# NVIDIA/spark-rapids-ml

Measured on NVIDIA H100. Metric: kmeans_fit_samples_per_sec, higher is better.
Workload: dtype f32

## Files before the change

profile_fused.py:

```python
from __future__ import annotations

import argparse
import json
import os
import sys

ROOT = os.path.dirname(os.path.abspath(__file__))
if ROOT not in sys.path:
    sys.path.insert(0, ROOT)

from bench_pca import _card

CONSUMER = ["X wait", "centre wait", "hand-off wait", "A load + split", "MMA issue + drain", "epilogue", "sort",
            "column sums"]
PRODUCER = ["X slot wait", "centre stage wait", "issue"]
TILE_ROWS = 128


def main() -> None:
    ap = argparse.ArgumentParser()
    ap.add_argument("--rows", type=int, default=10_000_000)
    ap.add_argument("--d", type=int, default=128)
    ap.add_argument("--k", type=int, default=64)
    ap.add_argument("--warmup", type=int, default=3)
    a = ap.parse_args()

    import numpy as np
    import torch

    from bench import make_blobs_device
    from spark_rapids_ml_b200 import _native

    dev = torch.device("cuda", 0)
    X, _ = make_blobs_device(torch, dev, a.rows, a.d, a.k, 0)
    C0 = X[: a.k].clone()
    with _native.Context(0) as ctx:
        ctx.set_option("kernel_path", 2)
        ctx.kmeans_lloyd(X, C0.clone(), a.warmup, -1.0)
        ctx.set_option("profile_fused", 1)
        ctx.kmeans_lloyd(X, C0.clone(), 1, -1.0)
        ctx.set_option("profile_fused", 0)
        prof = ctx.fused_profile().astype(np.float64)
    grid = prof.shape[0]
    ntiles = -(-a.rows // TILE_ROWS)
    tiles = np.array([len(range(b, ntiles, grid)) for b in range(grid)], dtype=np.float64)
    per_tile = prof / tiles[:, None, None]
    cons = per_tile[:, :8, :].mean(axis=(0, 1))
    prod = per_tile[:, 8, :3].mean(axis=0)
    rec = {"shape": {"n": a.rows, "d": a.d, "k": a.k}, "grid": grid, "tiles_per_cta": float(tiles.mean()),
           "consumer_cycles_per_tile": {nm: round(float(v)) for nm, v in zip(CONSUMER, cons)},
           "consumer_total": round(float(cons.sum())),
           "producer_cycles_per_tile": {nm: round(float(v)) for nm, v in zip(PRODUCER, prod)},
           "producer_total": round(float(prod.sum())), **_card()}
    print(f"{rec['gpu']}, power limit {rec['power_limit']}; grid {grid}, {rec['tiles_per_cta']:.1f} tiles per CTA")
    print("consumer warps (mean), cycles per tile:")
    for nm, v in rec["consumer_cycles_per_tile"].items():
        print(f"  {nm:20s} {v:8d}")
    print(f"  {'total':20s} {rec['consumer_total']:8d}")
    print("producer warp, cycles per tile:")
    for nm, v in rec["producer_cycles_per_tile"].items():
        print(f"  {nm:20s} {v:8d}")
    print(f"  {'total':20s} {rec['producer_total']:8d}")
    print(json.dumps(rec))


if __name__ == "__main__":
    main()
# ... 1 lines not shown
```

spark_rapids_ml_b200/csrc/b2k_ptx.cuh:

```cuda
#pragma once
__device__ __forceinline__ uint32_t smem_u32(const void* p) { return (uint32_t)__cvta_generic_to_shared(p); }

__device__ __forceinline__ void mbar_init(uint32_t bar, uint32_t count) {
  asm volatile("mbarrier.init.shared::cta.b64 [%0], %1;" ::"r"(bar), "r"(count) : "memory");
}
__device__ __forceinline__ void mbar_arrive(uint32_t bar) {
  asm volatile("mbarrier.arrive.shared::cta.b64 _, [%0];" ::"r"(bar) : "memory");
}
__device__ __forceinline__ void mbar_expect_tx(uint32_t bar, uint32_t bytes) {
  asm volatile("mbarrier.arrive.expect_tx.shared::cta.b64 _, [%0], %1;" ::"r"(bar), "r"(bytes) : "memory");
}
__device__ __forceinline__ uint32_t mbar_try_wait(uint32_t bar, uint32_t parity) {
  uint32_t ok;
  asm volatile(
      "{\n\t.reg .pred p;\n\t"
      "mbarrier.try_wait.parity.shared::cta.b64 p, [%1], %2, %3;\n\t"
      "selp.u32 %0, 1, 0, p;\n\t}"
      : "=r"(ok)
      : "r"(bar), "r"(parity), "r"(200000u)
      : "memory");
  return ok;
}
__device__ __forceinline__ void mbar_wait_nocall(uint32_t bar, uint32_t parity) {
  uint32_t spins = 0;
// ... 142 lines not shown
      : "+f"(d[0]), "+f"(d[1]), "+f"(d[2]), "+f"(d[3]), "+f"(d[4]), "+f"(d[5]), "+f"(d[6]), "+f"(d[7]), "+f"(d[8]), "+f"(d[9]), "+f"(d[10]), "+f"(d[11]), "+f"(d[12]), "+f"(d[13]), "+f"(d[14]), "+f"(d[15]), "+f"(d[16]), "+f"(d[17]), "+f"(d[18]), "+f"(d[19]), "+f"(d[20]), "+f"(d[21]), "+f"(d[22]), "+f"(d[23]), "+f"(d[24]), "+f"(d[25]), "+f"(d[26]), "+f"(d[27]), "+f"(d[28]), "+f"(d[29]), "+f"(d[30]), "+f"(d[31]), "+f"(d[32]), "+f"(d[33]), "+f"(d[34]), "+f"(d[35]), "+f"(d[36]), "+f"(d[37]), "+f"(d[38]), "+f"(d[39]), "+f"(d[40]), "+f"(d[41]), "+f"(d[42]), "+f"(d[43]), "+f"(d[44]), "+f"(d[45]), "+f"(d[46]), "+f"(d[47]), "+f"(d[48]), "+f"(d[49]), "+f"(d[50]), "+f"(d[51]), "+f"(d[52]), "+f"(d[53]), "+f"(d[54]), "+f"(d[55]), "+f"(d[56]), "+f"(d[57]), "+f"(d[58]), "+f"(d[59]), "+f"(d[60]), "+f"(d[61]), "+f"(d[62]), "+f"(d[63]), "+f"(d[64]), "+f"(d[65]), "+f"(d[66]), "+f"(d[67]), "+f"(d[68]), "+f"(d[69]), "+f"(d[70]), "+f"(d[71]), "+f"(d[72]), "+f"(d[73]), "+f"(d[74]), "+f"(d[75]), "+f"(d[76]), "+f"(d[77]), "+f"(d[78]), "+f"(d[79]), "+f"(d[80]), "+f"(d[81]), "+f"(d[82]), "+f"(d[83]), "+f"(d[84]), "+f"(d[85]), "+f"(d[86]), "+f"(d[87]), "+f"(d[88]), "+f"(d[89]), "+f"(d[90]), "+f"(d[91]), "+f"(d[92]), "+f"(d[93]), "+f"(d[94]), "+f"(d[95]), "+f"(d[96]), "+f"(d[97]), "+f"(d[98]), "+f"(d[99]), "+f"(d[100]), "+f"(d[101]), "+f"(d[102]), "+f"(d[103]), "+f"(d[104]), "+f"(d[105]), "+f"(d[106]), "+f"(d[107]), "+f"(d[108]), "+f"(d[109]), "+f"(d[110]), "+f"(d[111]), "+f"(d[112]), "+f"(d[113]), "+f"(d[114]), "+f"(d[115]), "+f"(d[116]), "+f"(d[117]), "+f"(d[118]), "+f"(d[119]), "+f"(d[120]), "+f"(d[121]), "+f"(d[122]), "+f"(d[123]), "+f"(d[124]), "+f"(d[125]), "+f"(d[126]), "+f"(d[127])
      : "l"(da), "l"(db), "r"(scale_d));
}
template <int N> __device__ __forceinline__ void wgmma_tf32(float (&d)[N / 2], uint64_t da, uint64_t db, uint32_t sd) {
  if constexpr (N == 16) wgmma_tf32_n16(d, da, db, sd);
  else if constexpr (N == 32) wgmma_tf32_n32(d, da, db, sd);
  else if constexpr (N == 64) wgmma_tf32_n64(d, da, db, sd);
  else if constexpr (N == 128) wgmma_tf32_n128(d, da, db, sd);
  else wgmma_tf32_n256(d, da, db, sd);
}

__device__ __forceinline__ void wgmma_tf32_rs_n16(float (&d)[8], const uint32_t (&a)[4], uint64_t db, uint32_t scale_d) {
  asm volatile(
      "{\n\t.reg .pred p;\n\t"
      "setp.ne.b32 p, %13, 0;\n\t"
      "wgmma.mma_async.sync.aligned.m64n16k8.f32.tf32.tf32 "
      "{%0, %1, %2, %3, %4, %5, %6, %7}, {%8, %9, %10, %11}, %12, p, 1, 1;\n\t}"
      : "+f"(d[0]), "+f"(d[1]), "+f"(d[2]), "+f"(d[3]), "+f"(d[4]), "+f"(d[5]), "+f"(d[6]), "+f"(d[7])
      : "r"(a[0]), "r"(a[1]), "r"(a[2]), "r"(a[3]), "l"(db), "r"(scale_d));
}
__device__ __forceinline__ void wgmma_tf32_rs_n32(float (&d)[16], const uint32_t (&a)[4], uint64_t db, uint32_t scale_d) {
  asm volatile(
      "{\n\t.reg .pred p;\n\t"
      "setp.ne.b32 p, %21, 0;\n\t"
      "wgmma.mma_async.sync.aligned.m64n32k8.f32.tf32.tf32 "
      "{%0, %1, %2, %3, %4, %5, %6, %7, %8, %9, %10, %11, %12, %13, %14, %15}, {%16, %17, %18, %19}, %20, p, 1, 1;\n\t}"
      : "+f"(d[0]), "+f"(d[1]), "+f"(d[2]), "+f"(d[3]), "+f"(d[4]), "+f"(d[5]), "+f"(d[6]), "+f"(d[7]), "+f"(d[8]), "+f"(d[9]), "+f"(d[10]), "+f"(d[11]), "+f"(d[12]), "+f"(d[13]), "+f"(d[14]), "+f"(d[15])
      : "r"(a[0]), "r"(a[1]), "r"(a[2]), "r"(a[3]), "l"(db), "r"(scale_d));
}
__device__ __forceinline__ void wgmma_tf32_rs_n64(float (&d)[32], const uint32_t (&a)[4], uint64_t db, uint32_t scale_d) {
  asm volatile(
      "{\n\t.reg .pred p;\n\t"
      "setp.ne.b32 p, %37, 0;\n\t"
      "wgmma.mma_async.sync.aligned.m64n64k8.f32.tf32.tf32 "
      "{%0, %1, %2, %3, %4, %5, %6, %7, %8, %9, %10, %11, %12, %13, %14, %15, %16, %17, %18, %19, %20, %21, %22, %23, %24, %25, %26, %27, %28, %29, %30, %31}, {%32, %33, %34, %35}, %36, p, 1, 1;\n\t}"
      : "+f"(d[0]), "+f"(d[1]), "+f"(d[2]), "+f"(d[3]), "+f"(d[4]), "+f"(d[5]), "+f"(d[6]), "+f"(d[7]), "+f"(d[8]), "+f"(d[9]), "+f"(d[10]), "+f"(d[11]), "+f"(d[12]), "+f"(d[13]), "+f"(d[14]), "+f"(d[15]), "+f"(d[16]), "+f"(d[17]), "+f"(d[18]), "+f"(d[19]), "+f"(d[20]), "+f"(d[21]), "+f"(d[22]), "+f"(d[23]), "+f"(d[24]), "+f"(d[25]), "+f"(d[26]), "+f"(d[27]), "+f"(d[28]), "+f"(d[29]), "+f"(d[30]), "+f"(d[31])
      : "r"(a[0]), "r"(a[1]), "r"(a[2]), "r"(a[3]), "l"(db), "r"(scale_d));
}
__device__ __forceinline__ void wgmma_tf32_rs_n128(float (&d)[64], const uint32_t (&a)[4], uint64_t db, uint32_t scale_d) {
  asm volatile(
      "{\n\t.reg .pred p;\n\t"
      "setp.ne.b32 p, %69, 0;\n\t"
      "wgmma.mma_async.sync.aligned.m64n128k8.f32.tf32.tf32 "
      "{%0, %1, %2, %3, %4, %5, %6, %7, %8, %9, %10, %11, %12, %13, %14, %15, %16, %17, %18, %19, %20, %21, %22, %23, %24, %25, %26, %27, %28, %29, %30, %31, %32, %33, %34, %35, %36, %37, %38, %39, %40, %41, %42, %43, %44, %45, %46, %47, %48, %49, %50, %51, %52, %53, %54, %55, %56, %57, %58, %59, %60, %61, %62, %63}, {%64, %65, %66, %67}, %68, p, 1, 1;\n\t}"
      : "+f"(d[0]), "+f"(d[1]), "+f"(d[2]), "+f"(d[3]), "+f"(d[4]), "+f"(d[5]), "+f"(d[6]), "+f"(d[7]), "+f"(d[8]), "+f"(d[9]), "+f"(d[10]), "+f"(d[11]), "+f"(d[12]), "+f"(d[13]), "+f"(d[14]), "+f"(d[15]), "+f"(d[16]), "+f"(d[17]), "+f"(d[18]), "+f"(d[19]), "+f"(d[20]), "+f"(d[21]), "+f"(d[22]), "+f"(d[23]), "+f"(d[24]), "+f"(d[25]), "+f"(d[26]), "+f"(d[27]), "+f"(d[28]), "+f"(d[29]), "+f"(d[30]), "+f"(d[31]), "+f"(d[32]), "+f"(d[33]), "+f"(d[34]), "+f"(d[35]), "+f"(d[36]), "+f"(d[37]), "+f"(d[38]), "+f"(d[39]), "+f"(d[40]), "+f"(d[41]), "+f"(d[42]), "+f"(d[43]), "+f"(d[44]), "+f"(d[45]), "+f"(d[46]), "+f"(d[47]), "+f"(d[48]), "+f"(d[49]), "+f"(d[50]), "+f"(d[51]), "+f"(d[52]), "+f"(d[53]), "+f"(d[54]), "+f"(d[55]), "+f"(d[56]), "+f"(d[57]), "+f"(d[58]), "+f"(d[59]), "+f"(d[60]), "+f"(d[61]), "+f"(d[62]), "+f"(d[63])
      : "r"(a[0]), "r"(a[1]), "r"(a[2]), "r"(a[3]), "l"(db), "r"(scale_d));
}
template <int N> __device__ __forceinline__ void wgmma_tf32_rs(float (&d)[N / 2], const uint32_t (&a)[4], uint64_t db, uint32_t sd) {
  if constexpr (N == 16) wgmma_tf32_rs_n16(d, a, db, sd);
  else if constexpr (N == 32) wgmma_tf32_rs_n32(d, a, db, sd);
  else if constexpr (N == 64) wgmma_tf32_rs_n64(d, a, db, sd);
  else wgmma_tf32_rs_n128(d, a, db, sd);
}
```

spark_rapids_ml_b200/csrc/b2k_wg.cuh:

```cuda
constexpr int WG_TM = B2K_FUSED_TILE_ROWS;
constexpr int WG_CHUNK = 32;
constexpr int WG_XBYTES = WG_TM * WG_CHUNK * 4;
constexpr int WG_NTHREADS = 384;
constexpr int WG_SMEM_LIMIT = 227 * 1024;
constexpr int WG_MISC = 7680;
constexpr int WG_M_CNORM = 256, WG_M_XN = 1280, WG_M_LAB = 1792, WG_M_FLAG = 2816, WG_M_COST = 2880, WG_M_SRT = 2944,
              WG_M_LIST = 3584;
constexpr int WG_MISC3 = 2368;
constexpr int WG_M3_XN = 768, WG_M3_SRT = 768, WG_M3_HIST = 1280, WG_M3_COST = 2304;
constexpr int WG_CL = 8;
constexpr int WG_NPROF = 8;
enum { WG_P_WX, WG_P_WC, WG_P_HAND, WG_P_SPLIT, WG_P_MMA, WG_P_EPI, WG_P_SORT, WG_P_SUMS };

template <int KP, int NCH, bool THREE, bool UPD>
struct WgCfg {
  static_assert(KP % 16 == 0 && KP >= 16 && KP <= 256, "KP");
  static_assert(!UPD || !THREE || (KP <= 128 && NCH <= 4), "3xTF32 covers k, d <= 128");
  static constexpr int SROWS = THREE ? KP : KP / WG_CL;
  static constexpr int DP = NCH * WG_CHUNK;
  static constexpr int NB = THREE ? 2 : 1;
  static constexpr int CBYTES = KP * WG_CHUNK * 4;
  static constexpr int CSTAGE = NB * CBYTES;
  static constexpr int MISC = THREE ? WG_MISC3 : WG_MISC;
  static constexpr int SUM_BYTES = UPD ? SROWS * DP * 4 + SROWS * 4 : 0;
  static constexpr int FIXED = SUM_BYTES + MISC;
  static constexpr int XMIN = UPD ? NCH : 2;
  static constexpr int XRES = UPD ? 2 * NCH : 2;
  static constexpr bool CRES = THREE && (WG_SMEM_LIMIT - FIXED - NCH * CSTAGE) / WG_XBYTES >= XRES;
  static constexpr int SC = CRES ? 1 : (WG_SMEM_LIMIT - FIXED - 2 * CSTAGE) / WG_XBYTES >= XMIN ? 2 : 1;
  static constexpr int C_BYTES = CRES ? NCH * CSTAGE : SC * CSTAGE;
  static constexpr int SX_RAW = (WG_SMEM_LIMIT - FIXED - C_BYTES) / WG_XBYTES;
  static constexpr int SX = SX_RAW > 12 ? 12 : SX_RAW;
  static_assert(SX >= XMIN && 2 * (SX + SC) * 8 + 16 <= WG_M_CNORM, "ring");
  static constexpr int OFF_X = 0;
  static constexpr int OFF_C = SX * WG_XBYTES;
  static constexpr int OFF_SUM = OFF_C + C_BYTES;
  static constexpr int OFF_MISC = OFF_SUM + (THREE ? (SUM_BYTES + 7) & ~7 : (SUM_BYTES + 1023) & ~1023);
  static constexpr int SMEM_BYTES = OFF_MISC + MISC;
  static_assert(SMEM_BYTES <= WG_SMEM_LIMIT, "smem");
  static_assert(!THREE || WG_M_CNORM + KP * 4 <= WG_M3_XN, "misc");
  static_assert(!THREE || WG_M3_HIST + 8 * KP <= WG_M3_COST, "misc");
};
static_assert(WgCfg<64, 4, true, true>::CRES, "cfg2 centres no longer resident");

struct WgArgs {
  int64_t n;
  int ntiles;
  int k;
  int d;
  const float* cnorm;
  int32_t* labels_out;
  float* mind_out;
  double* cost_partials;
  float* partials;
  int32_t* counts;
  const B2kLoopState* st;
  const float* X;
  const float* C32;
  const float* thr;
  const float2* xnorm;
  int2* fix_list;
  uint32_t* fix_masks;
  int32_t* fix_count;
  int seg_cap;
  int mask_cap;
  unsigned long long* rstat;
  long long* prof;
};

__device__ __forceinline__ void wg_merge2(uint32_t& a1, uint32_t& a2, uint32_t b1, uint32_t b2) {
  const uint32_t lo = min(a1, b1), hi = max(a1, b1);
  a2 = min(hi, min(a2, b2));
  a1 = lo;
}

template <int KP, int NCH, bool THREE, bool NC, bool UPD, bool PROF = false>
__global__ void __launch_bounds__(WG_NTHREADS, 1)
k_wg_assign(const __grid_constant__ CUtensorMap mapX, const __grid_constant__ CUtensorMap mapC0,
            const __grid_constant__ CUtensorMap mapC1, const WgArgs args) {
  using G = WgCfg<KP, NCH, THREE, UPD>;
  constexpr int R = KP / 2;
  constexpr int DP = G::DP;
  if (args.st != nullptr && args.st->done) return;

  extern __shared__ __align__(1024) uint8_t smem_raw[];
  const uint32_t base = smem_u32(smem_raw);
  if ((base & 1023u) != 0u) {
    if (threadIdx.x == 0) printf("b2k wgmma: dynamic shared memory base %u is not 1 KB aligned\n", base);
    __trap();
  }
  uint8_t* misc = smem_raw + G::OFF_MISC;
  const uint32_t bars = base + G::OFF_MISC;
  float* cnorm_s = reinterpret_cast<float*>(misc + WG_M_CNORM);
  float* xn_s = reinterpret_cast<float*>(misc + WG_M3_XN);
  int32_t* lab_s = reinterpret_cast<int32_t*>(misc + WG_M_LAB);
  uint8_t* hist_s = misc + WG_M3_HIST;
  int32_t* flag_s = reinterpret_cast<int32_t*>(misc + WG_M_FLAG);
  double* cost_s = reinterpret_cast<double*>(misc + (THREE ? WG_M3_COST : WG_M_COST));
  uint32_t* srt_s = reinterpret_cast<uint32_t*>(misc + (THREE ? WG_M3_SRT : WG_M_SRT));
  float* sum_s = reinterpret_cast<float*>(smem_raw + G::OFF_SUM);
  int32_t* cnt_s = reinterpret_cast<int32_t*>(sum_s + G::SROWS * DP);
  uint32_t* list_s = reinterpret_cast<uint32_t*>(misc + WG_M_LIST);
  auto xfull = [&](int s) -> uint32_t { return bars + 8u * (uint32_t)s; };
  auto xempty = [&](int s) -> uint32_t { return bars + 8u * (uint32_t)(G::SX + s); };
  auto cfull = [&](int s) -> uint32_t { return bars + 8u * (uint32_t)(2 * G::SX + s); };
  auto cempty = [&](int s) -> uint32_t { return bars + 8u * (uint32_t)(2 * G::SX + G::SC + s); };
  constexpr bool CLU = UPD && !THREE;
  const uint32_t ready_bar = bars + 8u * (uint32_t)(2 * G::SX + 2 * G::SC);
  const uint32_t done_bar = ready_bar + 8u;

  const int warp = threadIdx.x >> 5;
  const int lane = threadIdx.x & 31;
  long long pc[WG_NPROF] = {};
  long long tp = PROF ? clock64() : 0;
  auto mark = [&](int ph) {
    if constexpr (PROF) {
      const long long t = clock64();
      pc[ph] += t - tp;
      tp = t;
    }
  };
  auto prof_store = [&]() {
    if constexpr (PROF) {
      long long* o = args.prof + ((size_t)blockIdx.x * (WG_NTHREADS / 32) + warp) * WG_NPROF;
      for (int i = 0; i < WG_NPROF; ++i) o[i] = pc[i];
    }
  };
  if (threadIdx.x == 0) {
    for (int s = 0; s < G::SX; ++s) {
      mbar_init(xfull(s), 1);
      mbar_init(xempty(s), 8);
    }
    for (int s = 0; s < G::SC; ++s) {
      mbar_init(cfull(s), 1);
      mbar_init(cempty(s), 8);
    }
    if constexpr (CLU) {
      mbar_init(ready_bar, WG_CL);
      mbar_init(done_bar, WG_CL);
    }
    asm volatile("fence.mbarrier_init.release.cluster;" ::: "memory");
  }
  for (int j = threadIdx.x; j < KP; j += WG_NTHREADS) cnorm_s[j] = args.cnorm[j];
  if constexpr (UPD) {
    for (int i = threadIdx.x; i < G::SROWS * DP + G::SROWS; i += WG_NTHREADS) sum_s[i] = 0.f;
  }
  __syncthreads();
  uint32_t crank = 0;
  if constexpr (CLU) {
    crank = cluster_ctarank();
    cluster_sync_all();
  }

  const int b0 = (int)blockIdx.x - (int)crank;
  const int nit = b0 < args.ntiles ? (args.ntiles - 1 - b0) / (int)gridDim.x + 1 : 0;

  if (warp >= 8) {
    if constexpr (!THREE) asm volatile("setmaxnreg.dec.sync.aligned.u32 40;" ::: "memory");
    if (warp == 8 && elect_one()) {
      tma_prefetch_desc(&mapX);
      tma_prefetch_desc(&mapC0);
      if constexpr (THREE) tma_prefetch_desc(&mapC1);
      if constexpr (G::CRES) {
        mbar_expect_tx(cfull(0), (uint32_t)(NCH * G::CSTAGE));
        for (int c = 0; c < NCH; ++c) {
          const uint32_t cst = base + (uint32_t)(G::OFF_C + c * G::CSTAGE);
          tma_load_2d(cst, &mapC0, cfull(0), c * WG_CHUNK, 0);
          tma_load_2d(cst + G::CBYTES, &mapC1, cfull(0), c * WG_CHUNK, 0);
        }
      }
      for (int it = 0; it < nit; ++it) {
        const int tile = (int)blockIdx.x + it * (int)gridDim.x;
#pragma unroll 1
        for (int c = 0; c < NCH; ++c) {
          const int q = it * NCH + c;
          const int xs = q % G::SX, cs = q % G::SC;
          mark(WG_P_HAND);
          mbar_wait_nocall(xempty(xs), (uint32_t)((q / G::SX) & 1) ^ 1u);
          mark(WG_P_WX);
          mbar_expect_tx(xfull(xs), (uint32_t)WG_XBYTES);
          tma_load_2d(base + (uint32_t)(G::OFF_X + xs * WG_XBYTES), &mapX, xfull(xs), c * WG_CHUNK, tile * WG_TM);
          if constexpr (!G::CRES) {
            mark(WG_P_HAND);
            mbar_wait_nocall(cempty(cs), (uint32_t)((q / G::SC) & 1) ^ 1u);
            mark(WG_P_WC);
            const uint32_t cst = base + (uint32_t)(G::OFF_C + cs * G::CSTAGE);
            mbar_expect_tx(cfull(cs), (uint32_t)G::CSTAGE);
            tma_load_2d(cst, &mapC0, cfull(cs), c * WG_CHUNK, 0);
            if constexpr (THREE) tma_load_2d(cst + G::CBYTES, &mapC1, cfull(cs), c * WG_CHUNK, 0);
          }
        }
      }
      mark(WG_P_HAND);
      prof_store();
    }
    __syncwarp();
  } else {
    if constexpr (!THREE) asm volatile("setmaxnreg.inc.sync.aligned.u32 232;" ::: "memory");
    const int g = warp >> 2, wi = warp & 3, tw = threadIdx.x & 127;
    float acc[R];
#pragma unroll
    for (int i = 0; i < R; ++i) acc[i] = 0.f;
    double cost = 0.0;
    int seg_cnt = 0;
    unsigned long long n_flag = 0;
    float thr0 = 0.f, thr1 = 0.f, thr2 = 0.f, thr3 = 0.f;
    if constexpr (!THREE) {
      thr0 = args.thr[0];
      thr1 = args.thr[1];
      thr2 = args.thr[2];
      thr3 = args.thr[3];
    }
    if constexpr (THREE) {
      const uint32_t arow = (uint32_t)(g * 64 + wi * 16 + (lane >> 2)) * 128u + (uint32_t)(lane & 3) * 4u;
      const uint32_t asw = (uint32_t)(lane >> 2);
      constexpr bool PIPE = (G::CRES || G::SC > 1) && KP < 128;
      if constexpr (G::CRES) {
        mark(WG_P_EPI);
        if (nit > 0) mbar_wait_nocall(cfull(0), 0u);
        mark(WG_P_WC);
      }
      for (int it = 0; it < nit; ++it) {
        const int tile = (int)blockIdx.x + it * (int)gridDim.x;
        float xnp[4] = {0.f, 0.f, 0.f, 0.f};
#pragma unroll
        for (int c = 0; c < NCH; ++c) {
          const int q = it * NCH + c;
          const int xsl = q % G::SX, csl = q % G::SC;
          const uint32_t xs = base + (uint32_t)(G::OFF_X + xsl * WG_XBYTES);
          const uint32_t cs = base + (uint32_t)(G::OFF_C + (G::CRES ? c : csl) * G::CSTAGE);
          const uint8_t* xp = smem_raw + G::OFF_X + xsl * WG_XBYTES;
          mark(WG_P_EPI);
          mbar_wait_nocall(xfull(xsl), (uint32_t)((q / G::SX) & 1));
          mark(WG_P_WX);
          if constexpr (NC) {
#pragma unroll
            for (int i = 0; i < 4; ++i) {
              const float4 v = lds128(xs + (uint32_t)(g * (WG_XBYTES / 2) + (tw + 128 * i) * 16));
              xnp[i] = fmaf(v.w, v.w, fmaf(v.z, v.z, fmaf(v.y, v.y, fmaf(v.x, v.x, xnp[i]))));
            }
          }
          uint32_t ah[WG_CHUNK / 8][4], al[WG_CHUNK / 8][4];
#pragma unroll
          for (int ks = 0; ks < WG_CHUNK / 8; ++ks) {
#pragma unroll
            for (int e = 0; e < 4; ++e) {
              const uint32_t unit = (uint32_t)(2 * ks + (e >> 1));
              const float v = *reinterpret_cast<const float*>(xp + arow + (uint32_t)(e & 1) * 1024u + ((unit ^ asw) << 4));
              ah[ks][e] = rn_tf32_bits(v);
              al[ks][e] = rn_tf32_bits(v - __uint_as_float(ah[ks][e]));
            }
          }
#pragma unroll
          for (int ks = 0; ks < WG_CHUNK / 8; ++ks) {
            reg_fence(ah[ks]);
            reg_fence(al[ks]);
          }
          if constexpr (!UPD) {
            __syncwarp();
            if (lane == 0) mbar_arrive(xempty(xsl));
          }
          mark(WG_P_SPLIT);
          if constexpr (!G::CRES) {
            mbar_wait_nocall(cfull(csl), (uint32_t)((q / G::SC) & 1));
            mark(WG_P_WC);
          }
          wgmma_fence();
#pragma unroll
          for (int ks = 0; ks < WG_CHUNK / 8; ++ks) {
// ... 22 lines not shown
          mark(WG_P_MMA);
        }
        wgmma_wait0();
        if constexpr (PIPE && !G::CRES) {
          __syncwarp();
          if (lane == 0) mbar_arrive(cempty((it * NCH + NCH - 1) % G::SC));
        }
        reg_fence(acc);
        mark(WG_P_MMA);

        const int rr0 = g * 64 + wi * 16 + (lane >> 2);
        if constexpr (NC) {
#pragma unroll
          for (int i = 0; i < 4; ++i) {
            float v = xnp[i];
            v += __shfl_xor_sync(0xffffffffu, v, 1);
            v += __shfl_xor_sync(0xffffffffu, v, 2);
            v += __shfl_xor_sync(0xffffffffu, v, 4);
            if ((lane & 7) == 0) xn_s[g * 64 + (tw >> 3) + 16 * i] = v;
          }
          asm volatile("bar.sync %0, 128;" ::"r"(1 + g) : "memory");
        }
        float best[2] = {__int_as_float(0x7f800000), __int_as_float(0x7f800000)};
        int bj[2] = {0, 0};
#pragma unroll
        for (int i = 0; i < R; ++i) {
          const int h = (i >> 1) & 1;
          const int j = (i >> 2) * 8 + 2 * (lane & 3) + (i & 1);
          const float dist = fmaf(-2.f, acc[i], cnorm_s[j]);
          if (dist < best[h]) { best[h] = dist; bj[h] = j; }
        }
#pragma unroll
        for (int h = 0; h < 2; ++h) {
#pragma unroll
          for (int o = 1; o <= 2; o <<= 1) {
            const float ob = __shfl_xor_sync(0xffffffffu, best[h], o);
            const int oj = __shfl_xor_sync(0xffffffffu, bj[h], o);
            if (ob < best[h] || (ob == best[h] && oj < bj[h])) { best[h] = ob; bj[h] = oj; }
          }
          const int64_t grow = (int64_t)tile * WG_TM + rr0 + 8 * h;
          if ((lane & 3) == 0) {
            if (grow < args.n) {
              if (args.labels_out != nullptr) args.labels_out[grow] = bj[h];
              if constexpr (NC) {
                const float md = fmaxf(xn_s[rr0 + 8 * h] + best[h], 0.f);
                if (args.mind_out != nullptr) args.mind_out[grow] = md;
                cost += (double)md;
              }
            }
          }
        }
        mark(WG_P_EPI);
        if constexpr (UPD) {
          const int hq = lane & 3;
          const int64_t grow0 = (int64_t)tile * WG_TM + rr0;
          const uint32_t key = hq == 0   ? (grow0 < args.n ? (uint32_t)bj[0] : (uint32_t)KP)
                               : hq == 1 ? (grow0 + 8 < args.n ? (uint32_t)bj[1] : (uint32_t)KP)
                                         : 0x10000u + (uint32_t)lane;
          const bool own = hq < 2 && key < (uint32_t)KP;
          const uint32_t mk = __match_any_sync(0xffffffffu, key);
          const uint32_t lt = (1u << lane) - 1u;
          const int wr = hq == 0 ? __popc(mk & 0x11111111u & lt) : __popc(mk & 0x11111111u) + __popc(mk & 0x22222222u & lt);
          uint8_t* hist = hist_s + warp * KP;
          if (lane < KP / 4) reinterpret_cast<uint32_t*>(hist)[lane] = 0u;
          __syncwarp();
          if (own && wr == 0) hist[key] = (uint8_t)__popc(mk & 0x33333333u);
          mark(WG_P_SORT);
          asm volatile("bar.sync 3, 256;" ::: "memory");
          mark(WG_P_HAND);
          uint32_t tot = 0u, pre = 0u;
          if (lane < KP / 4) {
#pragma unroll
            for (int w = 0; w < 8; ++w) {
              const uint32_t v = reinterpret_cast<const uint32_t*>(hist_s + w * KP)[lane];
              tot += v;
              if (w < warp) pre += v;
            }
          }
          const int lsum = (int)((tot * 0x01010101u) >> 24);
          int incl = lsum;
#pragma unroll
          for (int o = 1; o < 32; o <<= 1) {
            const int v = __shfl_up_sync(0xffffffffu, incl, o);
            if (lane >= o) incl += v;
          }
          const int nv = __shfl_sync(0xffffffffu, incl, 31);
          const uint32_t first = tot * 0x01010100u + (uint32_t)(incl - lsum) * 0x01010101u + pre;
          const uint32_t fb = __shfl_sync(0xffffffffu, first, (int)(key >> 2) & 31);
          if (own) srt_s[((fb >> (8 * (key & 3u))) & 0xffu) + (uint32_t)wr] = (key << 16) | (uint32_t)(rr0 + 8 * hq);
          mark(WG_P_SORT);
          asm volatile("bar.sync 3, 256;" ::: "memory");
          mark(WG_P_HAND);
          int p0 = 128, p1 = 128;
          {
            const uint4 e4 = *reinterpret_cast<const uint4*>(srt_s + 4 * lane);
            const uint32_t ev[4] = {e4.x, e4.y, e4.z, e4.w};
            uint32_t prev = __shfl_up_sync(0xffffffffu, e4.w >> 16, 1);
#pragma unroll
            for (int i = 0; i < 4; ++i) {
              const int p = 4 * lane + i;
              const uint32_t l = ev[i] >> 16;
              if (p < nv && (p == 0 || l != prev)) {
                if (p >= 16 * warp && p0 == 128) p0 = p;
                if (p >= 16 * warp + 16 && p1 == 128) p1 = p;
              }
              prev = l;
            }
            p0 = min(__reduce_min_sync(0xffffffffu, p0), nv);
            p1 = min(__reduce_min_sync(0xffffffffu, p1), nv);
          }
          const bool act = lane < DP / 4;
          const uint8_t* xbase = smem_raw + G::OFF_X + ((it * NCH + (act ? lane >> 3 : 0)) % G::SX) * WG_XBYTES;
          const uint32_t unit = (uint32_t)(lane & 7);
          float4 a = make_float4(0.f, 0.f, 0.f, 0.f);
          int cur = -1, run = 0;
          auto flush = [&]() {
            if (act) {
              float4* sp = reinterpret_cast<float4*>(sum_s + cur * DP) + lane;
              float4 s = *sp;
              s.x += a.x;
              s.y += a.y;
              s.z += a.z;
              s.w += a.w;
              *sp = s;
            }
            if (lane == 0) cnt_s[cur] += run;
          };
#pragma unroll 1
          for (int i0 = p0; i0 < p1; i0 += 8) {
            uint32_t e[8];
            float4 x[8];
#pragma unroll
            for (int v = 0; v < 8; ++v) e[v] = i0 + v < p1 ? srt_s[i0 + v] : 0xffffffffu;
#pragma unroll
            for (int v = 0; v < 8; ++v) {
              const uint32_t r = e[v] & 127u;
              x[v] = *reinterpret_cast<const float4*>(xbase + r * 128u + ((unit ^ (r & 7u)) << 4));
            }
#pragma unroll
            for (int v = 0; v < 8; ++v) {
              if (e[v] == 0xffffffffu) break;
              const int l = (int)(e[v] >> 16);
              if (l != cur) {
                if (cur >= 0) flush();
                cur = l;
                a = make_float4(0.f, 0.f, 0.f, 0.f);
                run = 0;
              }
              a.x += x[v].x;
              a.y += x[v].y;
              a.z += x[v].z;
              a.w += x[v].w;
              ++run;
            }
          }
          if (cur >= 0) flush();
          __syncwarp();
          if (lane == 0) {
#pragma unroll
            for (int c = 0; c < NCH; ++c) mbar_arrive(xempty((it * NCH + c) % G::SX));
          }
          mark(WG_P_SUMS);
        }
      }
    } else {
      for (int it = 0; it < nit; ++it) {
        const int tile = (int)blockIdx.x + it * (int)gridDim.x;
        int prev_q = -1;
#pragma unroll 1
        for (int c = 0; c < NCH; ++c) {
          const int q = it * NCH + c;
          const int xsl = q % G::SX, csl = q % G::SC;
          const uint32_t xs = base + (uint32_t)(G::OFF_X + xsl * WG_XBYTES + g * (WG_XBYTES / 2));
          const uint32_t cs = base + (uint32_t)(G::OFF_C + csl * G::CSTAGE);
          mbar_wait_nocall(xfull(xsl), (uint32_t)((q / G::SX) & 1));
          mbar_wait_nocall(cfull(csl), (uint32_t)((q / G::SC) & 1));
          wgmma_fence();
#pragma unroll
          for (int ks = 0; ks < WG_CHUNK / 8; ++ks) {
            const uint64_t da = make_kmajor_sw128_desc(xs + ks * 32);
            const uint64_t db = make_kmajor_sw128_desc(cs + ks * 32);
            const uint32_t sd = (c | ks) != 0 ? 1u : 0u;
            wgmma_tf32<KP>(acc, da, db, sd);
          }
          wgmma_commit();
          if constexpr (G::SC == 1) {
            wgmma_wait0();
            __syncwarp();
            if (lane == 0) {
              mbar_arrive(cempty(csl));
              if constexpr (!UPD) mbar_arrive(xempty(xsl));
            }
          } else {
            wgmma_wait1();
            if (prev_q >= 0) {
              __syncwarp();
              if (lane == 0) {
                if constexpr (!UPD) mbar_arrive(xempty(prev_q % G::SX));
                mbar_arrive(cempty(prev_q % G::SC));
              }
            }
            prev_q = q;
          }
        }
        if constexpr (G::SC > 1) {
          wgmma_wait0();
          __syncwarp();
          if (lane == 0) {
            if constexpr (!UPD) mbar_arrive(xempty(prev_q % G::SX));
            mbar_arrive(cempty(prev_q % G::SC));
          }
        }
        reg_fence(acc);

        const int rr0 = g * 64 + wi * 16 + (lane >> 2);
// ... 157 lines not shown
#pragma unroll 1
            for (int c = 0; c < NCH; ++c) mbar_arrive(xempty((it * NCH + c) % G::SX));
          }
        }
        if constexpr (NC) {
#pragma unroll 1
          for (int r2 = 0; r2 < 16; ++r2) {
            const int row = warp * 16 + r2;
            const int lab = lab_s[pb * WG_TM + row];
            if (lab < 0) continue;
            const int64_t gr = (int64_t)tile * WG_TM + row;
            float sacc = 0.f;
#pragma unroll
            for (int t = 0; t < 2; ++t) {
              const int cc = lane * 4 + 128 * t;
              if (cc < args.d) {
                const float4 xv = __ldg(reinterpret_cast<const float4*>(args.X + (size_t)gr * args.d + cc));
                const float4 cv = __ldg(reinterpret_cast<const float4*>(args.C32 + (size_t)lab * args.d + cc));
                const float dx = xv.x - cv.x, dy = xv.y - cv.y, dz = xv.z - cv.z, dw = xv.w - cv.w;
                sacc = fmaf(dx, dx, fmaf(dy, dy, fmaf(dz, dz, fmaf(dw, dw, sacc))));
              }
            }
#pragma unroll
            for (int o = 16; o > 0; o >>= 1) sacc += __shfl_xor_sync(0xffffffffu, sacc, o);
            if (lane == 0) {
              if (args.mind_out != nullptr) args.mind_out[gr] = sacc;
              cost += (double)sacc;
            }
          }
        }
      }
    }
#pragma unroll
    for (int o = 16; o > 0; o >>= 1) cost += __shfl_xor_sync(0xffffffffu, cost, o);
    if (lane == 0) cost_s[warp] = cost;
    mark(WG_P_EPI);
    if (lane == 0) prof_store();
    if constexpr (!THREE) {
      if (threadIdx.x == 0) args.fix_count[blockIdx.x] = seg_cnt;
      if (args.rstat != nullptr) {
#pragma unroll
        for (int o = 16; o > 0; o >>= 1) n_flag += __shfl_xor_sync(0xffffffffu, n_flag, o);
        if (lane == 0 && n_flag != 0ull) atomicAdd(args.rstat + 0, n_flag);
      }
    }
  }
  __syncthreads();
  if (threadIdx.x == 0) {
    double c = 0.0;
    for (int w = 0; w < 8; ++w) c += cost_s[w];
    args.cost_partials[blockIdx.x] = c;
  }
  if constexpr (UPD && THREE) {
    const int kd = args.k * args.d;
    float* out = args.partials + (size_t)blockIdx.x * kd;
    for (int i = threadIdx.x; i < kd; i += WG_NTHREADS) out[i] = sum_s[(i / args.d) * DP + i % args.d];
    for (int l = threadIdx.x; l < args.k; l += WG_NTHREADS) args.counts[(size_t)blockIdx.x * args.k + l] = cnt_s[l];
  }
  if constexpr (CLU) {
    const size_t slot = (size_t)(blockIdx.x / WG_CL);
    const int l0 = (int)crank * G::SROWS;
    const int nl = min(G::SROWS, args.k - l0);
    for (int i = threadIdx.x; i < nl * args.d; i += WG_NTHREADS)
      args.partials[(slot * args.k + l0) * args.d + i] = sum_s[(i / args.d) * DP + i % args.d];
    for (int l = threadIdx.x; l < nl; l += WG_NTHREADS) args.counts[slot * args.k + l0 + l] = cnt_s[l];
    cluster_sync_all();
  }
}

template <int KP, int NCH, bool THREE>
int b2k_launch_wg(b2k_ctx* ctx, int grid, const CUtensorMap& mx, const CUtensorMap& m0, const CUtensorMap& m1,
                  const WgArgs& a, bool need_cost, bool do_update, cudaStream_t s) {
  int smem = 0;
  void (*kern)(CUtensorMap, CUtensorMap, CUtensorMap, WgArgs) = nullptr;
  if (do_update) {
    kern = k_wg_assign<KP, NCH, THREE, false, true>;
    smem = WgCfg<KP, NCH, THREE, true>::SMEM_BYTES;
  } else {
    kern = need_cost ? k_wg_assign<KP, NCH, THREE, true, false> : k_wg_assign<KP, NCH, THREE, false, false>;
    smem = WgCfg<KP, NCH, THREE, false>::SMEM_BYTES;
  }
  if constexpr (THREE) {
    if (a.prof != nullptr) {
      kern = do_update ? k_wg_assign<KP, NCH, THREE, false, true, true>
             : need_cost ? k_wg_assign<KP, NCH, THREE, true, false, true>
                         : k_wg_assign<KP, NCH, THREE, false, false, true>;
    }
  }
  B2K_CUDA_OK(ctx, cudaFuncSetAttribute(kern, cudaFuncAttributeMaxDynamicSharedMemorySize, smem));
  if (!THREE && do_update) {
    if (grid % WG_CL != 0) return b2k_fail(ctx, B2K_ERR_STATE, "fused kernel: grid is not a multiple of the cluster size");
    cudaLaunchConfig_t cfg{};
    cfg.gridDim = dim3((unsigned)grid);
    cfg.blockDim = dim3(WG_NTHREADS);
    cfg.dynamicSmemBytes = (size_t)smem;
    cfg.stream = s;
    cudaLaunchAttribute attr[1];
    attr[0].id = cudaLaunchAttributeClusterDimension;
    attr[0].val.clusterDim.x = WG_CL;
    attr[0].val.clusterDim.y = 1;
    attr[0].val.clusterDim.z = 1;
    cfg.attrs = attr;
    cfg.numAttrs = 1;
    B2K_CUDA_OK(ctx, cudaLaunchKernelEx(&cfg, kern, mx, m0, m1, a));
  } else {
    kern<<<grid, WG_NTHREADS, smem, s>>>(mx, m0, m1, a);
  }
  B2K_CUDA_OK(ctx, cudaGetLastError());
  return B2K_OK;
// ... 2 lines not shown
```

Measured before the change: 3.500 billion.

## Compute per-cluster sums via one-hot bf16 wgmma instead of sort-and-accumulate

Replaces the warp histogram, prefix-sum sort and scalar float4 accumulation of per-cluster row sums with a one-hot label matrix in shared memory, multiplied against X on tensor cores. X is split into three bf16 parts so the sums stay close to fp32 accuracy. Partial sums are kept in registers across tiles and written out once at the end, with counts kept via shared atomics. This moves the update work onto tensor cores and removes the serial run-length loop, at the cost of extra smem for one-hot buffers, more register pressure, and three bf16 MMAs per k-step.

```diff
diff --git a/profile_fused.py b/profile_fused.py
--- a/profile_fused.py
+++ b/profile_fused.py
@@ -11,8 +11,8 @@
 
 from bench_pca import _card
 
-CONSUMER = ["X wait", "centre wait", "hand-off wait", "A load + split", "MMA issue + drain", "epilogue", "sort",
-            "column sums"]
+CONSUMER = ["X wait", "centre wait", "hand-off wait", "A load + split", "MMA issue + drain", "epilogue",
+            "one-hot + counts", "sums"]
 PRODUCER = ["X slot wait", "centre stage wait", "issue"]
 TILE_ROWS = 128
 
diff --git a/spark_rapids_ml_b200/csrc/b2k_ptx.cuh b/spark_rapids_ml_b200/csrc/b2k_ptx.cuh
--- a/spark_rapids_ml_b200/csrc/b2k_ptx.cuh
+++ b/spark_rapids_ml_b200/csrc/b2k_ptx.cuh
@@ -218,3 +218,55 @@
   else if constexpr (N == 64) wgmma_tf32_rs_n64(d, a, db, sd);
   else wgmma_tf32_rs_n128(d, a, db, sd);
 }
+
+__device__ __forceinline__ void split3_bf16x2(float lo, float hi, uint32_t (&b)[3]) {
+#pragma unroll
+  for (int t = 0; t < 3; ++t) {
+    asm("cvt.rn.bf16x2.f32 %0, %1, %2;" : "=r"(b[t]) : "f"(hi), "f"(lo));
+    lo -= __uint_as_float(b[t] << 16);
+    hi -= __uint_as_float(b[t] & 0xffff0000u);
+  }
+}
+
+__device__ __forceinline__ void wgmma_bf16_rs_n16(float (&d)[8], const uint32_t (&a)[4], uint64_t db) {
+  asm volatile(
+      "{\n\t.reg .pred p;\n\t"
+      "setp.ne.b32 p, 1, 0;\n\t"
+      "wgmma.mma_async.sync.aligned.m64n16k16.f32.bf16.bf16 "
+      "{%0, %1, %2, %3, %4, %5, %6, %7}, {%8, %9, %10, %11}, %12, p, 1, 1, 0;\n\t}"
+      : "+f"(d[0]), "+f"(d[1]), "+f"(d[2]), "+f"(d[3]), "+f"(d[4]), "+f"(d[5]), "+f"(d[6]), "+f"(d[7])
+      : "r"(a[0]), "r"(a[1]), "r"(a[2]), "r"(a[3]), "l"(db));
+}
+__device__ __forceinline__ void wgmma_bf16_rs_n32(float (&d)[16], const uint32_t (&a)[4], uint64_t db) {
+  asm volatile(
+      "{\n\t.reg .pred p;\n\t"
+      "setp.ne.b32 p, 1, 0;\n\t"
+      "wgmma.mma_async.sync.aligned.m64n32k16.f32.bf16.bf16 "
+      "{%0, %1, %2, %3, %4, %5, %6, %7, %8, %9, %10, %11, %12, %13, %14, %15}, {%16, %17, %18, %19}, %20, p, 1, 1, 0;\n\t}"
+      : "+f"(d[0]), "+f"(d[1]), "+f"(d[2]), "+f"(d[3]), "+f"(d[4]), "+f"(d[5]), "+f"(d[6]), "+f"(d[7]), "+f"(d[8]), "+f"(d[9]), "+f"(d[10]), "+f"(d[11]), "+f"(d[12]), "+f"(d[13]), "+f"(d[14]), "+f"(d[15])
+      : "r"(a[0]), "r"(a[1]), "r"(a[2]), "r"(a[3]), "l"(db));
+}
+__device__ __forceinline__ void wgmma_bf16_rs_n64(float (&d)[32], const uint32_t (&a)[4], uint64_t db) {
+  asm volatile(
+      "{\n\t.reg .pred p;\n\t"
+      "setp.ne.b32 p, 1, 0;\n\t"
+      "wgmma.mma_async.sync.aligned.m64n64k16.f32.bf16.bf16 "
+      "{%0, %1, %2, %3, %4, %5, %6, %7, %8, %9, %10, %11, %12, %13, %14, %15, %16, %17, %18, %19, %20, %21, %22, %23, %24, %25, %26, %27, %28, %29, %30, %31}, {%32, %33, %34, %35}, %36, p, 1, 1, 0;\n\t}"
+      : "+f"(d[0]), "+f"(d[1]), "+f"(d[2]), "+f"(d[3]), "+f"(d[4]), "+f"(d[5]), "+f"(d[6]), "+f"(d[7]), "+f"(d[8]), "+f"(d[9]), "+f"(d[10]), "+f"(d[11]), "+f"(d[12]), "+f"(d[13]), "+f"(d[14]), "+f"(d[15]), "+f"(d[16]), "+f"(d[17]), "+f"(d[18]), "+f"(d[19]), "+f"(d[20]), "+f"(d[21]), "+f"(d[22]), "+f"(d[23]), "+f"(d[24]), "+f"(d[25]), "+f"(d[26]), "+f"(d[27]), "+f"(d[28]), "+f"(d[29]), "+f"(d[30]), "+f"(d[31])
+      : "r"(a[0]), "r"(a[1]), "r"(a[2]), "r"(a[3]), "l"(db));
+}
+__device__ __forceinline__ void wgmma_bf16_rs_n128(float (&d)[64], const uint32_t (&a)[4], uint64_t db) {
+  asm volatile(
+      "{\n\t.reg .pred p;\n\t"
+      "setp.ne.b32 p, 1, 0;\n\t"
+      "wgmma.mma_async.sync.aligned.m64n128k16.f32.bf16.bf16 "
+      "{%0, %1, %2, %3, %4, %5, %6, %7, %8, %9, %10, %11, %12, %13, %14, %15, %16, %17, %18, %19, %20, %21, %22, %23, %24, %25, %26, %27, %28, %29, %30, %31, %32, %33, %34, %35, %36, %37, %38, %39, %40, %41, %42, %43, %44, %45, %46, %47, %48, %49, %50, %51, %52, %53, %54, %55, %56, %57, %58, %59, %60, %61, %62, %63}, {%64, %65, %66, %67}, %68, p, 1, 1, 0;\n\t}"
+      : "+f"(d[0]), "+f"(d[1]), "+f"(d[2]), "+f"(d[3]), "+f"(d[4]), "+f"(d[5]), "+f"(d[6]), "+f"(d[7]), "+f"(d[8]), "+f"(d[9]), "+f"(d[10]), "+f"(d[11]), "+f"(d[12]), "+f"(d[13]), "+f"(d[14]), "+f"(d[15]), "+f"(d[16]), "+f"(d[17]), "+f"(d[18]), "+f"(d[19]), "+f"(d[20]), "+f"(d[21]), "+f"(d[22]), "+f"(d[23]), "+f"(d[24]), "+f"(d[25]), "+f"(d[26]), "+f"(d[27]), "+f"(d[28]), "+f"(d[29]), "+f"(d[30]), "+f"(d[31]), "+f"(d[32]), "+f"(d[33]), "+f"(d[34]), "+f"(d[35]), "+f"(d[36]), "+f"(d[37]), "+f"(d[38]), "+f"(d[39]), "+f"(d[40]), "+f"(d[41]), "+f"(d[42]), "+f"(d[43]), "+f"(d[44]), "+f"(d[45]), "+f"(d[46]), "+f"(d[47]), "+f"(d[48]), "+f"(d[49]), "+f"(d[50]), "+f"(d[51]), "+f"(d[52]), "+f"(d[53]), "+f"(d[54]), "+f"(d[55]), "+f"(d[56]), "+f"(d[57]), "+f"(d[58]), "+f"(d[59]), "+f"(d[60]), "+f"(d[61]), "+f"(d[62]), "+f"(d[63])
+      : "r"(a[0]), "r"(a[1]), "r"(a[2]), "r"(a[3]), "l"(db));
+}
+template <int N> __device__ __forceinline__ void wgmma_bf16_rs(float (&d)[N / 2], const uint32_t (&a)[4], uint64_t db) {
+  if constexpr (N == 16) wgmma_bf16_rs_n16(d, a, db);
+  else if constexpr (N == 32) wgmma_bf16_rs_n32(d, a, db);
+  else if constexpr (N == 64) wgmma_bf16_rs_n64(d, a, db);
+  else wgmma_bf16_rs_n128(d, a, db);
+}
diff --git a/spark_rapids_ml_b200/csrc/b2k_wg.cuh b/spark_rapids_ml_b200/csrc/b2k_wg.cuh
--- a/spark_rapids_ml_b200/csrc/b2k_wg.cuh
+++ b/spark_rapids_ml_b200/csrc/b2k_wg.cuh
@@ -6,11 +6,11 @@
 constexpr int WG_MISC = 7680;
 constexpr int WG_M_CNORM = 256, WG_M_XN = 1280, WG_M_LAB = 1792, WG_M_FLAG = 2816, WG_M_COST = 2880, WG_M_SRT = 2944,
               WG_M_LIST = 3584;
-constexpr int WG_MISC3 = 2368;
-constexpr int WG_M3_XN = 768, WG_M3_SRT = 768, WG_M3_HIST = 1280, WG_M3_COST = 2304;
+constexpr int WG_MISC3 = 1856;
+constexpr int WG_M3_XN = 768, WG_M3_CNT = 1280, WG_M3_COST = 1792;
 constexpr int WG_CL = 8;
 constexpr int WG_NPROF = 8;
-enum { WG_P_WX, WG_P_WC, WG_P_HAND, WG_P_SPLIT, WG_P_MMA, WG_P_EPI, WG_P_SORT, WG_P_SUMS };
+enum { WG_P_WX, WG_P_WC, WG_P_HAND, WG_P_SPLIT, WG_P_MMA, WG_P_EPI, WG_P_ONEHOT, WG_P_SUMS };
 
 template <int KP, int NCH, bool THREE, bool UPD>
 struct WgCfg {
@@ -22,7 +22,10 @@
   static constexpr int CBYTES = KP * WG_CHUNK * 4;
   static constexpr int CSTAGE = NB * CBYTES;
   static constexpr int MISC = THREE ? WG_MISC3 : WG_MISC;
-  static constexpr int SUM_BYTES = UPD ? SROWS * DP * 4 + SROWS * 4 : 0;
+  static constexpr int OH_BYTES = KP * WG_TM * 2;
+  static constexpr int NOH = KP == 128 ? 1 : 2;
+  static constexpr bool SSMEM = KP == 128 && DP > 64;
+  static constexpr int SUM_BYTES = !UPD ? 0 : THREE ? NOH * OH_BYTES + (SSMEM ? 32 * 256 * 4 : 0) : SROWS * DP * 4 + SROWS * 4;
   static constexpr int FIXED = SUM_BYTES + MISC;
   static constexpr int XMIN = UPD ? NCH : 2;
   static constexpr int XRES = UPD ? 2 * NCH : 2;
@@ -39,7 +42,7 @@
   static constexpr int SMEM_BYTES = OFF_MISC + MISC;
   static_assert(SMEM_BYTES <= WG_SMEM_LIMIT, "smem");
   static_assert(!THREE || WG_M_CNORM + KP * 4 <= WG_M3_XN, "misc");
-  static_assert(!THREE || WG_M3_HIST + 8 * KP <= WG_M3_COST, "misc");
+  static_assert(!THREE || WG_M3_CNT + 4 * KP <= WG_M3_COST, "misc");
 };
 static_assert(WgCfg<64, 4, true, true>::CRES, "cfg2 centres no longer resident");
 
@@ -94,12 +97,11 @@
   float* cnorm_s = reinterpret_cast<float*>(misc + WG_M_CNORM);
   float* xn_s = reinterpret_cast<float*>(misc + WG_M3_XN);
   int32_t* lab_s = reinterpret_cast<int32_t*>(misc + WG_M_LAB);
-  uint8_t* hist_s = misc + WG_M3_HIST;
   int32_t* flag_s = reinterpret_cast<int32_t*>(misc + WG_M_FLAG);
   double* cost_s = reinterpret_cast<double*>(misc + (THREE ? WG_M3_COST : WG_M_COST));
-  uint32_t* srt_s = reinterpret_cast<uint32_t*>(misc + (THREE ? WG_M3_SRT : WG_M_SRT));
+  uint32_t* srt_s = reinterpret_cast<uint32_t*>(misc + WG_M_SRT);
   float* sum_s = reinterpret_cast<float*>(smem_raw + G::OFF_SUM);
-  int32_t* cnt_s = reinterpret_cast<int32_t*>(sum_s + G::SROWS * DP);
+  int32_t* cnt_s = THREE ? reinterpret_cast<int32_t*>(misc + WG_M3_CNT) : reinterpret_cast<int32_t*>(sum_s + G::SROWS * DP);
   uint32_t* list_s = reinterpret_cast<uint32_t*>(misc + WG_M_LIST);
   auto xfull = [&](int s) -> uint32_t { return bars + 8u * (uint32_t)s; };
   auto xempty = [&](int s) -> uint32_t { return bars + 8u * (uint32_t)(G::SX + s); };
@@ -111,11 +113,11 @@
 
   const int warp = threadIdx.x >> 5;
   const int lane = threadIdx.x & 31;
-  long long pc[WG_NPROF] = {};
-  long long tp = PROF ? clock64() : 0;
+  uint32_t pc[WG_NPROF] = {};
+  uint32_t tp = PROF ? (uint32_t)clock() : 0u;
   auto mark = [&](int ph) {
     if constexpr (PROF) {
-      const long long t = clock64();
+      const uint32_t t = (uint32_t)clock();
       pc[ph] += t - tp;
       tp = t;
     }
@@ -123,7 +125,7 @@
   auto prof_store = [&]() {
     if constexpr (PROF) {
       long long* o = args.prof + ((size_t)blockIdx.x * (WG_NTHREADS / 32) + warp) * WG_NPROF;
-      for (int i = 0; i < WG_NPROF; ++i) o[i] = pc[i];
+      for (int i = 0; i < WG_NPROF; ++i) o[i] = (long long)pc[i];
     }
   };
   if (threadIdx.x == 0) {
@@ -142,7 +144,12 @@
     asm volatile("fence.mbarrier_init.release.cluster;" ::: "memory");
   }
   for (int j = threadIdx.x; j < KP; j += WG_NTHREADS) cnorm_s[j] = args.cnorm[j];
-  if constexpr (UPD) {
+  if constexpr (UPD && THREE) {
+    for (int i = threadIdx.x; i < G::SUM_BYTES / 16; i += WG_NTHREADS)
+      reinterpret_cast<uint4*>(smem_raw + G::OFF_SUM)[i] = make_uint4(0u, 0u, 0u, 0u);
+    for (int j = threadIdx.x; j < KP; j += WG_NTHREADS) cnt_s[j] = 0;
+    asm volatile("fence.proxy.async.shared::cta;" ::: "memory");
+  } else if constexpr (UPD) {
     for (int i = threadIdx.x; i < G::SROWS * DP + G::SROWS; i += WG_NTHREADS) sum_s[i] = 0.f;
   }
   __syncthreads();
@@ -215,6 +222,23 @@
       const uint32_t arow = (uint32_t)(g * 64 + wi * 16 + (lane >> 2)) * 128u + (uint32_t)(lane & 3) * 4u;
       const uint32_t asw = (uint32_t)(lane >> 2);
       constexpr bool PIPE = (G::CRES || G::SC > 1) && KP < 128;
+      constexpr bool SCEN = KP == 128;
+      constexpr bool SCOL = DP > 64 && !SCEN;
+      constexpr int MB = SCEN && DP > 64 ? 2 : 1;
+      constexpr int NS = SCEN ? KP / 2 : KP;
+      constexpr int RS = NS / 2;
+      constexpr int SKS = SCOL || SCEN ? 8 : 4;
+      constexpr int SSL = SCOL && PIPE ? 2 : 1;
+      float stot[UPD ? RS : 1];
+#pragma unroll
+      for (int i = 0; i < (UPD ? RS : 1); ++i) stot[i] = 0.f;
+      float* sslot = reinterpret_cast<float*>(smem_raw + G::OFF_SUM + G::NOH * G::OH_BYTES) + threadIdx.x;
+      const int scol = (SCOL ? 64 * g : 0) + 16 * wi + (lane >> 2);
+      const bool scol_ok = scol < DP;
+      const int srow0 = SCOL || SCEN ? 0 : 64 * g;
+      const uint32_t srow = (uint32_t)(2 * (lane & 3));
+      const uint32_t soff = srow * 128u + ((((uint32_t)(scol % WG_CHUNK) / 4u) ^ srow) << 4) + (uint32_t)(scol % 4) * 4u;
+      int oh_old[2] = {-1, -1}, oh_new[2] = {-1, -1};
       if constexpr (G::CRES) {
         mark(WG_P_EPI);
         if (nit > 0) mbar_wait_nocall(cfull(0), 0u);
@@ -343,115 +367,109 @@
         }
         mark(WG_P_EPI);
         if constexpr (UPD) {
-          const int hq = lane & 3;
-          const int64_t grow0 = (int64_t)tile * WG_TM + rr0;
-          const uint32_t key = hq == 0   ? (grow0 < args.n ? (uint32_t)bj[0] : (uint32_t)KP)
-                               : hq == 1 ? (grow0 + 8 < args.n ? (uint32_t)bj[1] : (uint32_t)KP)
-                                         : 0x10000u + (uint32_t)lane;
-          const bool own = hq < 2 && key < (uint32_t)KP;
-          const uint32_t mk = __match_any_sync(0xffffffffu, key);
-          const uint32_t lt = (1u << lane) - 1u;
-          const int wr = hq == 0 ? __popc(mk & 0x11111111u & lt) : __popc(mk & 0x11111111u) + __popc(mk & 0x22222222u & lt);
-          uint8_t* hist = hist_s + warp * KP;
-          if (lane < KP / 4) reinterpret_cast<uint32_t*>(hist)[lane] = 0u;
-          __syncwarp();
-          if (own && wr == 0) hist[key] = (uint8_t)__popc(mk & 0x33333333u);
-          mark(WG_P_SORT);
+          const uint32_t ohb = (uint32_t)(G::OFF_SUM + (it % G::NOH) * G::OH_BYTES);
+          if ((lane & 3) == 0) {
+#pragma unroll
+            for (int h = 0; h < 2; ++h) {
+              const int r = rr0 + 8 * h;
+              auto at = [&](int j) {
+                return reinterpret_cast<uint16_t*>(smem_raw + ohb + (r >> 6) * (KP * 128) + j * 128 +
+                                                   ((((r & 63) >> 3) ^ (j & 7)) << 4) + (r & 7) * 2);
+              };
+              const int stale = G::NOH == 2 ? oh_old[h] : oh_new[h];
+              if (stale >= 0) *at(stale) = 0;
+              const bool v = (int64_t)tile * WG_TM + r < args.n;
+              if (v) {
+                *at(bj[h]) = 0x3f80;
+                atomicAdd(cnt_s + bj[h], 1);
+              }
+              oh_old[h] = oh_new[h];
+              oh_new[h] = v ? bj[h] : -1;
+            }
+          }
+          asm volatile("fence.proxy.async.shared::cta;" ::: "memory");
+          mark(WG_P_ONEHOT);
           asm volatile("bar.sync 3, 256;" ::: "memory");
           mark(WG_P_HAND);
-          uint32_t tot = 0u, pre = 0u;
-          if (lane < KP / 4) {
-#pragma unroll
-            for (int w = 0; w < 8; ++w) {
-              const uint32_t v = reinterpret_cast<const uint32_t*>(hist_s + w * KP)[lane];
-              tot += v;
-              if (w < warp) pre += v;
-            }
-          }
-          const int lsum = (int)((tot * 0x01010101u) >> 24);
-          int incl = lsum;
-#pragma unroll
-          for (int o = 1; o < 32; o <<= 1) {
-            const int v = __shfl_up_sync(0xffffffffu, incl, o);
-            if (lane >= o) incl += v;
-          }
-          const int nv = __shfl_sync(0xffffffffu, incl, 31);
-          const uint32_t first = tot * 0x01010100u + (uint32_t)(incl - lsum) * 0x01010101u + pre;
-          const uint32_t fb = __shfl_sync(0xffffffffu, first, (int)(key >> 2) & 31);
-          if (own) srt_s[((fb >> (8 * (key & 3u))) & 0xffu) + (uint32_t)wr] = (key << 16) | (uint32_t)(rr0 + 8 * hq);
-          mark(WG_P_SORT);
+          const uint32_t ohk = base + ohb + (uint32_t)(SCOL ? 0 : SCEN ? g * (64 * 128) : g * (KP * 128));
+#pragma unroll
+          for (int mb = 0; mb < MB; ++mb) {
+          const uint8_t* xsum = smem_raw + G::OFF_X + ((it * NCH + scol / WG_CHUNK + 2 * mb) % G::SX) * WG_XBYTES;
+          float sacc[RS];
+#pragma unroll
+          for (int i = 0; i < RS; ++i) sacc[i] = 0.f;
+#pragma unroll
+          for (int s0 = 0; s0 < SKS; s0 += SSL) {
+            uint32_t a[SSL][3][4];
+#pragma unroll
+            for (int ss = 0; ss < SSL; ++ss) {
+#pragma unroll
+              for (int e = 0; e < 4; ++e) {
+                const uint8_t* xp = xsum + (srow0 + 16 * (s0 + ss) + 8 * (e >> 1)) * 128;
+                const uint32_t o = soff ^ ((e & 1) ? 0x20u : 0u);
+                const float lo = scol_ok ? *reinterpret_cast<const float*>(xp + o) : 0.f;
+                const float hi = scol_ok ? *reinterpret_cast<const float*>(xp + (o ^ 0x90u)) : 0.f;
+                uint32_t b[3];
+                split3_bf16x2(lo, hi, b);
+#pragma unroll
+                for (int t = 0; t < 3; ++t) a[ss][t][e] = b[2 - t];
+              }
+            }
+#pragma unroll
+            for (int ss = 0; ss < SSL; ++ss)
+#pragma unroll
+              for (int t = 0; t < 3; ++t) reg_fence(a[ss][t]);
+            if (s0 + SSL == SKS && mb == MB - 1) {
+              __syncwarp();
+              if (lane == 0) {
+#pragma unroll
+                for (int c = 0; c < NCH; ++c) mbar_arrive(xempty((it * NCH + c) % G::SX));
+              }
+            }
+            wgmma_fence();
+#pragma unroll
+            for (int ss = 0; ss < SSL; ++ss) {
+              const int st = s0 + ss;
+              const uint64_t db = make_kmajor_sw128_desc(ohk + (uint32_t)((st >> 2) * (KP * 128) + (st & 3) * 32));
+#pragma unroll
+              for (int t = 0; t < 3; ++t) wgmma_bf16_rs<NS>(sacc, a[ss][t], db);
+            }
+            wgmma_commit();
+            wgmma_wait1();
+          }
+          wgmma_wait0();
+          reg_fence(sacc);
+#pragma unroll
+          for (int i = 0; i < RS; ++i) {
+            if (mb == 0) stot[i] += sacc[i];
+            else sslot[i * 256] = (it == 0 ? 0.f : sslot[i * 256]) + sacc[i];
+          }
+          }
+          if constexpr (G::NOH == 1) asm volatile("bar.sync 3, 256;" ::: "memory");
+          mark(WG_P_SUMS);
+        }
+      }
+      if constexpr (UPD) {
+        float* stage = reinterpret_cast<float*>(smem_raw + G::OFF_SUM);
+        if constexpr (!SCOL && !SCEN) {
           asm volatile("bar.sync 3, 256;" ::: "memory");
-          mark(WG_P_HAND);
-          int p0 = 128, p1 = 128;
-          {
-            const uint4 e4 = *reinterpret_cast<const uint4*>(srt_s + 4 * lane);
-            const uint32_t ev[4] = {e4.x, e4.y, e4.z, e4.w};
-            uint32_t prev = __shfl_up_sync(0xffffffffu, e4.w >> 16, 1);
-#pragma unroll
-            for (int i = 0; i < 4; ++i) {
-              const int p = 4 * lane + i;
-              const uint32_t l = ev[i] >> 16;
-              if (p < nv && (p == 0 || l != prev)) {
-                if (p >= 16 * warp && p0 == 128) p0 = p;
-                if (p >= 16 * warp + 16 && p1 == 128) p1 = p;
-              }
-              prev = l;
-            }
-            p0 = min(__reduce_min_sync(0xffffffffu, p0), nv);
-            p1 = min(__reduce_min_sync(0xffffffffu, p1), nv);
-          }
-          const bool act = lane < DP / 4;
-          const uint8_t* xbase = smem_raw + G::OFF_X + ((it * NCH + (act ? lane >> 3 : 0)) % G::SX) * WG_XBYTES;
-          const uint32_t unit = (uint32_t)(lane & 7);
-          float4 a = make_float4(0.f, 0.f, 0.f, 0.f);
-          int cur = -1, run = 0;
-          auto flush = [&]() {
-            if (act) {
-              float4* sp = reinterpret_cast<float4*>(sum_s + cur * DP) + lane;
-              float4 s = *sp;
-              s.x += a.x;
-              s.y += a.y;
-              s.z += a.z;
-              s.w += a.w;
-              *sp = s;
-            }
-            if (lane == 0) cnt_s[cur] += run;
-          };
-#pragma unroll 1
-          for (int i0 = p0; i0 < p1; i0 += 8) {
-            uint32_t e[8];
-            float4 x[8];
-#pragma unroll
-            for (int v = 0; v < 8; ++v) e[v] = i0 + v < p1 ? srt_s[i0 + v] : 0xffffffffu;
-#pragma unroll
-            for (int v = 0; v < 8; ++v) {
-              const uint32_t r = e[v] & 127u;
-              x[v] = *reinterpret_cast<const float4*>(xbase + r * 128u + ((unit ^ (r & 7u)) << 4));
-            }
-#pragma unroll
-            for (int v = 0; v < 8; ++v) {
-              if (e[v] == 0xffffffffu) break;
-              const int l = (int)(e[v] >> 16);
-              if (l != cur) {
-                if (cur >= 0) flush();
-                cur = l;
-                a = make_float4(0.f, 0.f, 0.f, 0.f);
-                run = 0;
-              }
-              a.x += x[v].x;
-              a.y += x[v].y;
-              a.z += x[v].z;
-              a.w += x[v].w;
-              ++run;
-            }
-          }
-          if (cur >= 0) flush();
-          __syncwarp();
-          if (lane == 0) {
-#pragma unroll
-            for (int c = 0; c < NCH; ++c) mbar_arrive(xempty((it * NCH + c) % G::SX));
-          }
-          mark(WG_P_SUMS);
+          if (g == 1) {
+#pragma unroll
+            for (int i = 0; i < RS; ++i) stage[i * 128 + tw] = stot[i];
+          }
+          asm volatile("bar.sync 3, 256;" ::: "memory");
+        }
+        if (SCOL || SCEN || g == 0) {
+          float* out = args.partials + (size_t)blockIdx.x * args.k * args.d;
+#pragma unroll
+          for (int mb = 0; mb < MB; ++mb)
+#pragma unroll
+            for (int i = 0; i < RS; ++i) {
+              const int col = scol + 64 * mb + 8 * ((i >> 1) & 1);
+              const int j = (SCEN ? 64 * g : 0) + (i >> 2) * 8 + 2 * (lane & 3) + (i & 1);
+              const float v = mb == 1 ? (nit > 0 ? sslot[i * 256] : 0.f) : SCOL || SCEN ? stot[i] : stot[i] + stage[i * 128 + tw];
+              if (col < args.d && j < args.k) out[(size_t)j * args.d + col] = v;
+            }
         }
       }
     } else {
@@ -715,9 +733,6 @@
     args.cost_partials[blockIdx.x] = c;
   }
   if constexpr (UPD && THREE) {
-    const int kd = args.k * args.d;
-    float* out = args.partials + (size_t)blockIdx.x * kd;
-    for (int i = threadIdx.x; i < kd; i += WG_NTHREADS) out[i] = sum_s[(i / args.d) * DP + i % args.d];
     for (int l = threadIdx.x; l < args.k; l += WG_NTHREADS) args.counts[(size_t)blockIdx.x * args.k + l] = cnt_s[l];
   }
   if constexpr (CLU) {
```

Result: faster. 3.799 billion, median of 6 (+8.5%).
